# wangtong627/COR

Measured on AMD Instinct MI355X. Metric: query triplets/sec (forward + similarity + top-k), higher is better.
Workload: dtype bf16

## Files before the change

cor_amd/_native.py:

```python
from __future__ import annotations

import ctypes as C
import os

_HERE = os.path.dirname(os.path.abspath(__file__))
LIB_PATH = os.environ.get("COR_AMD_LIB") or os.path.join(_HERE, "csrc", "libcor_amd.so")

F32, BF16, F16, BF16X3 = 0, 1, 2, 3
I8 = 4
ACT_NONE, ACT_GELU_ERF, ACT_RELU, ACT_SIGMOID, ACT_GELU_TANH = 0, 1, 2, 3, 4
EINVAL, ENOSUPPORT = -1, -2
TOPK_FORCE_LISTS, TOPK_NO_FALLBACK, TOPK_FORCE_GLOBAL_THRESHOLD, TOPK_WAVE_FINAL = 1, 2, 8, 16
TOPK_KMAX = 256
FILTER_EQ, FILTER_NE = 0, 1
MERGE_NMAX = 4096
EXPAND_SEGMAX = 16
RERANK_SEGMAX = 16
DIVERSIFY_SEGMAX = 16
DIFFUSE_NMAX, DIFFUSE_KDMAX, DIFFUSE_SEGMAX = 256, 32, 16
CLUSTER_SEGMAX, KMEANS_KMAX = 16, 16384
IVF_NPROBE_MAX = 256
FUSE_PMAX = 16
FUSE_RRF, FUSE_SUM, FUSE_MAX = 0, 1, 2
FUSE_NORM_NONE, FUSE_NORM_MINMAX = 0, 1
FUSE_MISSING_ZERO, FUSE_MISSING_FLOOR = 0, 1
ORDER_REVERSE = 1 << 30
GEMM_KERNEL_SCALAR, GEMM_KERNEL_MASK, GEMM_EPILOGUE_VEC = 32, 0xff, 1 << 8
KERNEL_ROWLANE, KERNEL_FEWQ, KERNEL_FLASH_MFMA, KERNEL_FLASH_PIPELINED, KERNEL_WINDOW_BLOCK = 1, 2, 3, 4, 5
import numpy as _np
Q_PRESCALE_HD64 = float(_np.float32(0.125) * _np.float32(1.4426950408889634))

_p, _i, _l, _f, _ll = C.c_void_p, C.c_int, C.c_long, C.c_float, C.c_longlong

SIGNATURES = {
    "cor_version": [],
    "cor_gemm": [_p, _l, _p, _l, _i, _p, _l, _i, _i, _i, _i, _p, _i, _p, _p, _l, _i, _i, _p],
    "cor_gemm_kernel_id": [_p, _l, _p, _l, _i, _p, _l, _i, _i, _i, _i, _p, _i, _p, _p, _l, _i, _i],
    "cor_layernorm": [_p, _i, _p, _i, _p, _p, _i, _i, _f, _i, _p],
    "cor_attention": [_p, _l, _l, _p, _l, _l, _p, _l, _l, _i, _p, _l, _l, _i, _i, _i, _i, _i, _i, _f, _p],
    "cor_attention_f32": [_p, _l, _l, _p, _l, _l, _p, _l, _l, _p, _l, _l, _i, _i, _i, _i, _i, _i, _f, _p],
    "cor_attention_kernel_id": [_i, _i, _i, _i, _i, _i],
    "cor_sam_attention": [_p, _i, _p, _i, _p, _p, _p, _i, _i, _i, _i, _i, _f, _i, _p],
    "cor_patchify": [_p, _p, _i, _i, _i, _i, _i, _i, _i, _p],
    "cor_im2col3x3": [_p, _i, _p, _i, _i, _i, _i, _p],
    "cor_add": [_p, _i, _p, _i, _p, _i, _l, _l, _p],
    "cor_copy_rows": [_p, _l, _i, _p, _l, _i, _i, _i, _p],
    "cor_split_x3": [_p, _l, _p, _l, _l, _i, _i, _p],
    "cor_tokens_to_nchw": [_p, _i, _p, _i, _i, _i, _p],
    "cor_nchw_to_tokens": [_p, _p, _i, _i, _i, _i, _p],
    "cor_l2norm_rows": [_p, _i, _p, _i, _i, _i, _f, _p],
    "cor_embed_tokens": [_p, _p, _p, _p, _i, _i, _i, _i, _p],
    "cor_bilinear": [_p, _p, _i, _i, _i, _i, _i, _i, _p],
    "cor_conv3x3s2_small": [_p, _i, _p, _p, _p, _i, _i, _i, _i, _i, _p],
    "cor_dwconv7x7": [_p, _p, _p, _p, _i, _i, _i, _i, _i, _p],
    "cor_adapter_pool": [_p, _p, _p, _i, _i, _i, _i, _p],
    "cor_masked_pool": [_p, _i, _p, _p, _i, _i, _i, _i, _i, _p],
    "cor_region_pool": [_p, _p, _p, _p, _i, _i, _i, _i, _i, _i, _i, _p],
    "cor_fuse_gate": [_p, _p, _p, _p, _p, _i, _i, _p],
    "cor_fuse_mix": [_p, _p, _p, _i, _i, _p],
    "cor_dense_pe": [_p, _p, _i, _i, _p],
# ... 100 lines not shown
```

cor_amd/csrc/common.h:

```cpp
#pragma once
#include <hip/hip_runtime.h>
#include <atomic>
#include <stdint.h>

#include "../../include/cor_amd.h"

typedef uint16_t bf16_t;

typedef float f32x4 __attribute__((ext_vector_type(4)));
typedef unsigned int u32x4 __attribute__((ext_vector_type(4)));
typedef float f32x16 __attribute__((ext_vector_type(16)));
typedef __bf16 bf16x8 __attribute__((ext_vector_type(8)));

#define COR_CHECK_LAUNCH()                                  \
  do {                                                      \
    hipError_t e__ = hipGetLastError();                     \
    if (e__ != hipSuccess) return (int)e__;                 \
  } while (0)

__device__ __forceinline__ float bf2f(bf16_t v) { return __uint_as_float(((uint32_t)v) << 16); }
__device__ __forceinline__ bf16_t f2bf(float f) {
  __bf16 b = (__bf16)f;
  return __builtin_bit_cast(uint16_t, b);
}
// ... 80 lines not shown
__device__ __forceinline__ float sigmoid_f(float x) { return 1.0f / (1.0f + __expf(-x)); }

__device__ __forceinline__ float apply_act(float v, int act) {
  switch (act) {
    case COR_ACT_GELU_ERF: return gelu_erf_f(v);
    case COR_ACT_RELU: return fmaxf(v, 0.0f);
    case COR_ACT_SIGMOID: return 1.0f / (1.0f + expf(-v));
    case COR_ACT_GELU_TANH: return gelu_tanh_f(v);
    default: return v;
  }
}

__device__ __forceinline__ float wave_sum(float v) {
#pragma unroll
  for (int o = 32; o > 0; o >>= 1) v += __shfl_xor(v, o, 64);
  return v;
}
__device__ __forceinline__ float wave_max(float v) {
#pragma unroll
  for (int o = 32; o > 0; o >>= 1) v = fmaxf(v, __shfl_xor(v, o, 64));
  return v;
}

__device__ __forceinline__ int xcd_remap(int bid, int nwg) {
  const int xcd = bid & 7, q = nwg >> 3, r = nwg & 7;
  return (xcd < r ? xcd * (q + 1) : r * (q + 1) + (xcd - r) * q) + (bid >> 3);
}

__device__ __forceinline__ void glds16(const void* gsrc, unsigned lds_dst) {
  unsigned keep;
  asm volatile("s_mov_b32 %0, m0\n\ts_mov_b32 m0, %2\n\ts_nop 0\n\tglobal_load_lds_dwordx4 %1, off\n\ts_mov_b32 m0, %0"
               : "=&s"(keep) : "v"(gsrc), "s"(lds_dst) : "memory");
}

__device__ __forceinline__ void glds16_so(const void* sbase, unsigned voff, unsigned lds_dst) {
  unsigned keep;
  asm volatile("s_mov_b32 %0, m0\n\ts_mov_b32 m0, %3\n\ts_nop 0\n\tglobal_load_lds_dwordx4 %1, %2\n\ts_mov_b32 m0, %0"
               : "=&s"(keep) : "v"(voff), "s"(sbase), "s"(lds_dst) : "memory");
}

__device__ __forceinline__ void glds16_so_pair4k(const void* sbase, unsigned voff0_plus2k, unsigned voff1_minus2k, unsigned lds_dst_plus2k) {
  unsigned keep;
  asm volatile("s_mov_b32 %0, m0\n\ts_mov_b32 m0, %4\n\ts_nop 0\n\t"
               "global_load_lds_dwordx4 %1, %3 offset:-2048\n\tglobal_load_lds_dwordx4 %2, %3 offset:2048\n\ts_mov_b32 m0, %0"
               : "=&s"(keep) : "v"(voff0_plus2k), "v"(voff1_minus2k), "s"(sbase), "s"(lds_dst_plus2k) : "memory");
}
// ... 35 lines not shown
```

cor_amd/csrc/gemm.hip:

```cpp
#include "common.h"

#ifdef COR_PROBES
#define COR_DBG(g_, bit_) ((g_).dbg & (bit_))
#else
#define COR_DBG(g_, bit_) 0
#endif
#ifndef COR_GEMM_DEFAULT_BIG
#define COR_GEMM_DEFAULT_BIG 2
#endif

namespace {

struct GemmArgs {
  const char* A; const char* W; char* C;
  long lda_b, ldw_b;
  long ldc;
  int M, N, Kb;
  int tm, tn;
  const float* bias; const float* col_scale; const float* residual;
  long ldr; int res_row_mod; int act;
  int group_m;
  unsigned long long* stamps;
  int dbg;
  int vec_epi;
  int rev;
  int nt_c;
  int order;
};

template <typename TA> struct Mfma;
template <> struct Mfma<float> {
  static __device__ __forceinline__ void run(const uint4& a, const uint4& b, f32x16& acc) {
    acc = __builtin_amdgcn_mfma_f32_32x32x2f32(__uint_as_float(a.x), __uint_as_float(b.x), acc, 0, 0, 0);
    acc = __builtin_amdgcn_mfma_f32_32x32x2f32(__uint_as_float(a.y), __uint_as_float(b.y), acc, 0, 0, 0);
    acc = __builtin_amdgcn_mfma_f32_32x32x2f32(__uint_as_float(a.z), __uint_as_float(b.z), acc, 0, 0, 0);
    acc = __builtin_amdgcn_mfma_f32_32x32x2f32(__uint_as_float(a.w), __uint_as_float(b.w), acc, 0, 0, 0);
  }
};
template <> struct Mfma<bf16_t> {
  static __device__ __forceinline__ void run(const uint4& a, const uint4& b, f32x16& acc) {
    acc = __builtin_amdgcn_mfma_f32_32x32x16_bf16(__builtin_bit_cast(bf16x8, a), __builtin_bit_cast(bf16x8, b), acc, 0, 0, 0);
  }
};

__device__ __forceinline__ void mfma16_bf16(const uint4& a, const uint4& b, f32x4& acc) {
  acc = __builtin_amdgcn_mfma_f32_16x16x32_bf16(__builtin_bit_cast(bf16x8, a), __builtin_bit_cast(bf16x8, b), acc, 0, 0, 0);
}

constexpr int ROWB = 128;

template <int ACT, typename TO = float> __device__ __forceinline__ float act_ct(float v) {
// ... 639 lines not shown
#pragma unroll
        for (int i = 0; i < 8; ++i)
#pragma unroll
          for (int j = 0; j < 4; ++j) t += acc16[i][j][0] + acc16[i][j][3];
      } else {
#pragma unroll
        for (int i = 0; i < MI; ++i)
#pragma unroll
          for (int j = 0; j < NJ; ++j) t += acc[i][j][0] + acc[i][j][15];
      }
      if (t == 1.2345f) ((float*)g.C)[tid] = t;
    } else
    switch (g.act) {
      case COR_ACT_GELU_ERF: COR_EPI(COR_ACT_GELU_ERF) break;
      case COR_ACT_RELU: COR_EPI(COR_ACT_RELU) break;
      case COR_ACT_SIGMOID: COR_EPI(COR_ACT_SIGMOID) break;
      case COR_ACT_GELU_TANH: COR_EPI(COR_ACT_GELU_TANH) break;
      default: COR_EPI(COR_ACT_NONE) break;
    }
#undef COR_EPI
#ifdef COR_PROBES
    if (g.stamps && blockIdx.x == 0 && tid == 0) { g.stamps[(qi - 1) * 16 + 15] = __builtin_readcyclecounter(); g.stamps[(qi - 1) * 16 + 14] = __builtin_amdgcn_s_memrealtime(); }
#endif
    if (Ln < 0) break;
    L = Ln;
    stores_pending = !COR_DBG(g, 2);
  }
}

template <typename TA, typename TO>
__global__ void __launch_bounds__(256) gemm_nt_small(const TA* A, long lda, const TA* W, long ldw, TO* C, long ldc,
                                                     int M, int N, int K, const float* bias, int act,
                                                     const float* col_scale, const float* residual, long ldr,
                                                     int res_row_mod) {
  __shared__ float As[32][33], Ws[32][33];
  const int tx = threadIdx.x & 31, ty = threadIdx.x >> 5;
  const int m0 = blockIdx.y * 32, n0 = blockIdx.x * 32;
  float acc[4] = {0, 0, 0, 0};
  for (int k0 = 0; k0 < K; k0 += 32) {
#pragma unroll
    for (int i = 0; i < 4; ++i) {
      const int rrow = ty + 8 * i, k = k0 + tx;
      As[rrow][tx] = (m0 + rrow < M && k < K) ? ld<TA>(A + (long)(m0 + rrow) * lda + k) : 0.0f;
      Ws[rrow][tx] = (n0 + rrow < N && k < K) ? ld<TA>(W + (long)(n0 + rrow) * ldw + k) : 0.0f;
    }
    __syncthreads();
#pragma unroll 8
    for (int kk = 0; kk < 32; ++kk) {
      const float w = Ws[tx][kk];
// ... 49 lines not shown
  if (cfg == 0) {
    cfg = (k128 && M >= 512 && N >= 64) ? ((N <= 256 && K >= 2048 && M >= 65536) ? 9 : COR_GEMM_DEFAULT_BIG) : 1;
    if (k128 && M < 512 && N >= 64) cfg = 4;
    if (cfg == 2 && (long)cdiv(M, 128) * cdiv(N, 128) < 256) cfg = 4;
    else if (cfg == 2 && (long)cdiv(M, 128) * cdiv(N, 128) < 512) cfg = 3;
    if (sizeof(TA) == 2 && k128 && !col_scale && (long)cdiv(M, 256) * cdiv(N, 256) >= 140 && 4L * N >= 3L * 256 * cdiv(N, 256) && K >= 256) cfg = 13;
  }
  if (!k128 && (cfg == 2 || cfg == 3 || cfg == 4)) cfg = 1;
  if (cfg == 13 || cfg == 14) {
    const long c_bytes = (((long)M - 1) * ldc + N) * (long)sizeof(TO);
    const bool ok = sizeof(TA) == 2 && k128 && vec_epi && !col_scale && N % 8 == 0 && c_bytes < (1L << 32) - 64 && !(sizeof(TO) == 2 && residual) &&
                    (long)M * lda_b < (1L << 32) && (long)N * ldw_b < (1L << 32);
    if (!ok) cfg = k128 ? 2 : 1;
    else return {cfg, vec_epi};
  }
  if (!k128 && cfg >= 9) cfg = 1;
  if (!(cfg == 9 || cfg == 2 || cfg == 3 || cfg == 4)) cfg = 1;
  return {cfg, vec_epi};
}

template <typename TA, typename TO>
int launch_gemm(const void* A, long lda, const void* W, long ldw, void* C, long ldc, int M, int N, int K,
                const float* bias, int act, const float* col_scale, const float* residual, long ldr, int res_row_mod,
                int cfg_arg, hipStream_t s) {
  const int g_gemm_dbg = (cfg_arg & ~COR_ORDER_REVERSE) >> 8;
  const long esz = sizeof(TA);
  const GemmRoute route = gemm_route<TA, TO>(A, lda, W, ldw, C, ldc, M, N, K, bias, col_scale, residual, ldr, cfg_arg);
  if (route.kernel == COR_GEMM_KERNEL_SCALAR) {
    hipLaunchKernelGGL((gemm_nt_small<TA, TO>), dim3(cdiv(N, 32), cdiv(M, 32)), dim3(256), 0, s, (const TA*)A, lda,
                       (const TA*)W, ldw, (TO*)C, ldc, M, N, K, bias, act, col_scale, residual, ldr, res_row_mod);
    COR_CHECK_LAUNCH();
    return 0;
  }
  GemmArgs g;
  g.A = (const char*)A; g.W = (const char*)W; g.C = (char*)C;
  g.lda_b = lda * esz; g.ldw_b = ldw * esz; g.ldc = ldc;
  g.M = M; g.N = N; g.Kb = (int)(K * esz);
  g.stamps = nullptr;
#ifdef COR_PROBES
  if (g_gemm_dbg & 0x100000) { g.stamps = (unsigned long long*)col_scale; col_scale = nullptr; }
#endif
  g.bias = bias; g.col_scale = col_scale; g.residual = residual; g.ldr = ldr; g.res_row_mod = res_row_mod; g.act = act;
  g.dbg = g_gemm_dbg & 0x3fefff; g.rev = (cfg_arg & COR_ORDER_REVERSE) ? 1 : 0;
  g.order = 1;
  g.nt_c = (sizeof(TO) == 2 && !residual) ? 1 : 0;
  g.group_m = ((g_gemm_dbg >> 4) & 0xff) ? ((g_gemm_dbg >> 4) & 0xff) : 8;
  g.vec_epi = route.vec_epi;
  const int cfg = route.kernel;
  if (cfg == 13 || cfg == 14) {
    if constexpr (sizeof(TA) == 2) {
      g.tm = cdiv(g.M, 256); g.tn = cdiv(g.N, 256);
      g.order = g.tn <= 4 ? 1 : 0;
      if (g_gemm_dbg & 0x1000) g.order ^= 1;
      static DevOnce once_a;
      const int n_cu = cor_device_cus();
      cor_max_dyn_lds((const void*)gemm_pp<TO, false>, 163840, once_a);
#ifdef COR_PROBES
      static DevOnce once_b;
      cor_max_dyn_lds((const void*)gemm_pp<TO, true>, 163840, once_b);
#endif
      const int total = g.tm * g.tn;
      int blocks = n_cu - (n_cu & 7);
      if (total < blocks) blocks = ((total + 7) / 8) * 8;
#ifdef COR_PROBES
      if (cfg == 14) hipLaunchKernelGGL((gemm_pp<TO, true>), dim3(blocks), dim3(512), 163840, s, g);
      else
#endif
      hipLaunchKernelGGL((gemm_pp<TO, false>), dim3(blocks), dim3(512), 163840, s, g);
      COR_CHECK_LAUNCH();
      return 0;
    }
  }
  switch (cfg) {
    case 9: return launch_tile<TA, TO, 256, 128, 4, 2, true, 3>(g, s);
    case 2: return launch_tile<TA, TO, 128, 128, 2, 2, true>(g, s);
    case 3: return launch_tile<TA, TO, 128, 64, 2, 2, true>(g, s);
    case 4: return launch_tile<TA, TO, 64, 64, 2, 2, true>(g, s);
    default: return launch_tile<TA, TO, 128, 128, 2, 2, false>(g, s);
  }
}

int gemm_check_args(const void* A, long lda, const void* W, long ldw, int& ab_dtype, const void* C, long ldc, int c_dtype, int M, int N, int& K,
                    const float* residual, long ldr, int cfg) {
  if (!A || !W || !C || M <= 0 || N <= 0 || K <= 0 || lda < K || ldw < K || ldc < N) return COR_EINVAL;
  {
    const int sel = cfg & 0xff;
// ... 23 lines not shown
  hipStream_t s = (hipStream_t)stream;
  if (ab_dtype == COR_F32 && c_dtype == COR_F32)
    return launch_gemm<float, float>(A, lda, W, ldw, C, ldc, M, N, K, bias, act, col_scale, residual, ldr, res_row_mod, cfg, s);
  if (ab_dtype == COR_BF16 && c_dtype == COR_BF16)
    return launch_gemm<bf16_t, bf16_t>(A, lda, W, ldw, C, ldc, M, N, K, bias, act, col_scale, residual, ldr, res_row_mod, cfg, s);
  if (ab_dtype == COR_BF16 && c_dtype == COR_F32)
    return launch_gemm<bf16_t, float>(A, lda, W, ldw, C, ldc, M, N, K, bias, act, col_scale, residual, ldr, res_row_mod, cfg, s);
  return launch_gemm<float, bf16_t>(A, lda, W, ldw, C, ldc, M, N, K, bias, act, col_scale, residual, ldr, res_row_mod, cfg, s);
}

extern "C" int cor_gemm_kernel_id(const void* A, long lda, const void* W, long ldw, int ab_dtype, const void* C, long ldc, int c_dtype,
                                  int M, int N, int K, const float* bias, int act, const float* col_scale,
                                  const float* residual, long ldr, int res_row_mod, int cfg) {
  (void)act; (void)res_row_mod;
  const int rc = gemm_check_args(A, lda, W, ldw, ab_dtype, C, ldc, c_dtype, M, N, K, residual, ldr, cfg);
  if (rc) return rc;
  GemmRoute r;
  if (ab_dtype == COR_F32 && c_dtype == COR_F32) r = gemm_route<float, float>(A, lda, W, ldw, C, ldc, M, N, K, bias, col_scale, residual, ldr, cfg);
  else if (ab_dtype == COR_BF16 && c_dtype == COR_BF16) r = gemm_route<bf16_t, bf16_t>(A, lda, W, ldw, C, ldc, M, N, K, bias, col_scale, residual, ldr, cfg);
  else if (ab_dtype == COR_BF16 && c_dtype == COR_F32) r = gemm_route<bf16_t, float>(A, lda, W, ldw, C, ldc, M, N, K, bias, col_scale, residual, ldr, cfg);
  else r = gemm_route<float, bf16_t>(A, lda, W, ldw, C, ldc, M, N, K, bias, col_scale, residual, ldr, cfg);
  return r.kernel | (r.vec_epi ? COR_GEMM_EPILOGUE_VEC : 0);
}
```

cor_amd/csrc/rows.hip:

```cpp
#include "common.h"

namespace {

template <typename TI, typename TO, int MAXV>
__global__ void __launch_bounds__(256) layernorm_kernel(const TI* x, TO* y, const float* w, const float* b, int rows, int C,
                                                        float eps, int act, int rev) {
  const int lane = threadIdx.x & 63;
  const int row = (rev ? (int)gridDim.x - 1 - (int)blockIdx.x : (int)blockIdx.x) * 4 + (threadIdx.x >> 6);
  if (row >= rows) return;
  const TI* xr = x + (long)row * C;
  const int nv = C >> 2;
  f32x4 v[MAXV];
  float s = 0.f;
#pragma unroll
  for (int i = 0; i < MAXV; ++i) {
    const int j = lane + 64 * i;
    if (j < nv) { v[i] = ld4<TI>(xr + 4 * j); s += v[i][0] + v[i][1] + v[i][2] + v[i][3]; }
  }
  const float mean = wave_sum(s) / C;
  float q = 0.f;
#pragma unroll
  for (int i = 0; i < MAXV; ++i) {
    const int j = lane + 64 * i;
    if (j < nv) {
// ... 1 lines not shown
      for (int e = 0; e < 4; ++e) { const float d = v[i][e] - mean; q += d * d; }
    }
  }
  const float rstd = 1.0f / sqrtf(wave_sum(q) / C + eps);
#pragma unroll
  for (int i = 0; i < MAXV; ++i) {
    const int j = lane + 64 * i;
    if (j < nv) {
      const f32x4 wv = *(const f32x4*)(w + 4 * j), bv = *(const f32x4*)(b + 4 * j);
      f32x4 o;
#pragma unroll
      for (int e = 0; e < 4; ++e) o[e] = apply_act((v[i][e] - mean) * rstd * wv[e] + bv[e], act);
      st4_row<TO>(y, row, C, 4 * j, o);
    }
  }
}

template <typename TI, typename TO, int NV, bool NT>
__global__ void __launch_bounds__(256) layernorm_half_kernel(const TI* x, TO* y, const float* w, const float* b, int rows, int C,
                                                             float eps, int act, int rev) {
  const int lane = threadIdx.x & 31;
  const int row = (rev ? (int)gridDim.x - 1 - (int)blockIdx.x : (int)blockIdx.x) * 8 + (threadIdx.x >> 5);
  if (row >= rows) return;
  const TI* xr = x + (long)row * C;
  f32x4 v[NV];
  float s = 0.f;
#pragma unroll
  for (int i = 0; i < NV; ++i) {
    if constexpr (NT && sizeof(TI) == 4) v[i] = __builtin_nontemporal_load((const f32x4*)(xr + 4 * (lane + 32 * i)));
    else v[i] = ld4<TI>(xr + 4 * (lane + 32 * i));
    s += (v[i][0] + v[i][1]) + (v[i][2] + v[i][3]);
  }
  auto hsum = [](float t) {
#pragma unroll
    for (int o = 16; o > 0; o >>= 1) t += __shfl_xor(t, o, 64);
    return t;
  };
  const float mean = hsum(s) / C;
  float q = 0.f;
#pragma unroll
  for (int i = 0; i < NV; ++i)
#pragma unroll
    for (int e = 0; e < 4; ++e) { const float d = v[i][e] - mean; q += d * d; }
  const float rstd = 1.0f / sqrtf(hsum(q) / C + eps);
#pragma unroll
  for (int i = 0; i < NV; ++i) {
    const int j = lane + 32 * i;
    const f32x4 wv = *(const f32x4*)(w + 4 * j), bv = *(const f32x4*)(b + 4 * j);
    f32x4 o;
#pragma unroll
    for (int e = 0; e < 4; ++e) o[e] = apply_act((v[i][e] - mean) * rstd * wv[e] + bv[e], act);
    st4_row<TO>(y, row, C, 4 * j, o);
  }
}

#ifdef COR_PROBES
template <int NV, bool WRITE_X>
__global__ void __launch_bounds__(256) layernorm_delta_probe(float* x, const bf16_t* dl, bf16_t* y, const float* w, const float* b, int rows, int C, float eps) {
  const int lane = threadIdx.x & 31;
  const int row = ((int)gridDim.x - 1 - (int)blockIdx.x) * 8 + (threadIdx.x >> 5);
  if (row >= rows) return;
  float* xr = x + (long)row * C;
  const bf16_t* dr = dl + (long)row * C;
  f32x4 v[NV];
  float s = 0.f;
#pragma unroll
  for (int i = 0; i < NV; ++i) {
    v[i] = __builtin_nontemporal_load((const f32x4*)(xr + 4 * (lane + 32 * i)));
    const f32x4 d = ld4<bf16_t>(dr + 4 * (lane + 32 * i));
    v[i] += d;
    if (WRITE_X) *(f32x4*)(xr + 4 * (lane + 32 * i)) = v[i];
    s += (v[i][0] + v[i][1]) + (v[i][2] + v[i][3]);
  }
  auto hsum = [](float t) {
#pragma unroll
    for (int o = 16; o > 0; o >>= 1) t += __shfl_xor(t, o, 64);
// ... 375 lines not shown
```

cor_amd/engine.py:

```python
from __future__ import annotations

import math

import torch

from . import _native as nat
from . import ops
from .ops import ACT_NONE, ACT_GELU_ERF, ACT_RELU, ACT_SIGMOID, ACT_GELU_TANH, X3

F32 = torch.float32


def _round_up(x, m):
    return (x + m - 1) // m * m


class _Packer:

    def __init__(self, sd: dict, T: torch.dtype):
        dev = next(iter(sd.values())).device
        if dev.type != "cuda":
            raise RuntimeError("cor_amd: the model must live on a GPU (model.to('cuda')); there is no CPU path")
        self.sd, self.T, self.W = sd, T, {}

# ... 137 lines not shown

def pack(sd: dict, scfg: dict, gcfg: dict, mask_pooling: str, T: torch.dtype, Q=None) -> dict:
    pk = _Packer(sd, T)
    pkq = pk if Q is None or Q == T else _Packer(sd, Q)
    pack_sam_encoder(pk, scfg)
    pack_prompt_encoder(pk)
    pack_siglip(pkq, gcfg)
    pack_support_head(pkq, mask_pooling)
    pack_mask_decoder(pk)
    if pkq is not pk:
        pk.W.update(pkq.W)
    return pk.W


def _lin(W, p, a, out_dtype, act=ACT_NONE, residual=None, col_scale=None, out=None, reverse=False, x3=False):
    return ops.gemm(a, W[p + "weight"], out_dtype=out_dtype, bias=W[p + "bias"], act=act, residual=residual,
                    col_scale=col_scale, out=out, reverse=reverse, x3=x3)


def _ln(W, p, x, eps, out_dtype, act=ACT_NONE, reverse=False):
    return ops.layernorm(x, W[p + "weight"], W[p + "bias"], eps, out_dtype=out_dtype, act=act, reverse=reverse)


def _gelu(kind):
    return ACT_GELU_ERF if kind == "erf" else ACT_GELU_TANH


def sam_encoder(W, img, cfg, T, p="image_encoder."):
    B = img.shape[0]
    g, d, H = cfg["img"] // cfg["patch"], cfg["dim"], cfg["heads"]
    assert img.shape[1:] == (3, cfg["img"], cfg["img"]), f"SAM input must be [B,3,{cfg['img']},{cfg['img']}], got {tuple(img.shape)}"
    cols = ops.patchify(img, cfg["patch"], W[p + "patch.K"], T)
    x = ops.gemm(cols, W[p + "patch_embed.proj.weight"], out_dtype=F32, bias=W[p + "patch_embed.proj.bias"],
                 residual=W[p + "pos_embed"], res_row_mod=g * g)
    del cols
    for i in range(cfg["depth"]):
        b = f"{p}blocks.{i}."
        win = 0 if i in cfg["global_idx"] else cfg["window"]
        h = _ln(W, b + "norm1.", x, 1e-6, T, reverse=True)
        qkv = _lin(W, b + "attn.qkv.", h, T)
        a = ops.sam_attention(qkv, W[b + "attn.pad_row"], W[b + "attn.rel_pos_h"], W[b + "attn.rel_pos_w"], B, H, g, win,
                              q_prescale=W[b + "attn.q_prescale"], reverse=True)
        del qkv
        _lin(W, b + "attn.proj.", a, F32, residual=x, out=x)
        h = _ln(W, b + "norm2.", x, 1e-6, T, reverse=True)
        m = _lin(W, b + "mlp.lin1.", h, T, act=ACT_GELU_ERF)
        _lin(W, b + "mlp.lin2.", m, F32, residual=x, out=x)
        del h, a, m
    y = ops.gemm(ops.cast(x, T), W[p + "neck.0.weight"], out_dtype=F32)
    y = _ln(W, p + "neck.1.", y, 1e-6, T)
    y = ops.gemm(ops.im2col3x3(y, B, g, g), W[p + "neck.2.weight"], out_dtype=F32)
    return _ln(W, p + "neck.3.", y, 1e-6, F32)


def _vit_mha(qkv, N, Tn, heads, D, T):
    hd = D // heads
    if T == X3:
        return ops.attention_f32(qkv[:, 0:D], qkv[:, D:2 * D], qkv[:, 2 * D:3 * D], N, heads, Tn, Tn, hd, hd ** -0.5, out_dtype=X3)
    return ops.attention(qkv[:, 0:D], qkv[:, D:2 * D], qkv[:, 2 * D:3 * D], N, heads, Tn, Tn, hd, hd ** -0.5, out_dtype=T)


def _qkv_dtype(T):
    return F32 if T == X3 else T


def siglip_vision(W, img, g, T, p="support_branch.siglip.model.visual.trunk."):
    N = img.shape[0]
    D, P = g["dim"], (g["image"] // g["patch"]) ** 2
    x3 = T == X3
    assert img.shape[1:] == (3, g["image"], g["image"]), f"SigLIP input must be [N,3,{g['image']},{g['image']}], got {tuple(img.shape)}"
    cols = ops.patchify(img, g["patch"], W[p + "patch.K"], T)
    x = ops.gemm(cols, W[p + "patch_embed.proj.weight"], out_dtype=F32, bias=W[p + "patch_embed.proj.bias"],
                 residual=W[p + "pos_embed"], res_row_mod=P, x3=x3)
    act = _gelu(g.get("v_gelu", g.get("gelu", "erf")))
    for i in range(g["depth"]):
        b = f"{p}blocks.{i}."
        h = _ln(W, b + "norm1.", x, 1e-6, T)
        qkv = _lin(W, b + "attn.qkv.", h, _qkv_dtype(T), x3=x3)
        a = _vit_mha(qkv, N, P, g["heads"], D, T)
        _lin(W, b + "attn.proj.", a, F32, residual=x, out=x, x3=x3)
        h = _ln(W, b + "norm2.", x, 1e-6, T)
        m = _lin(W, b + "mlp.fc1.", h, T, act=act, x3=x3)
        _lin(W, b + "mlp.fc2.", m, F32, residual=x, out=x, x3=x3)
    return _ln(W, p + "norm.", x, 1e-6, F32)


def siglip_text(W, tokens, g, T, p="support_branch.siglip.model.text."):
    N, ctx = tokens.shape
    D = g["dim"]
    x3 = T == X3
    x = ops.embed_tokens(tokens.contiguous(), W[p + "token_embedding.weight"], W[p + "positional_embedding"])
    act = _gelu(g.get("t_gelu", g.get("gelu", "erf")))
    for i in range(g["t_depth"]):
        b = f"{p}transformer.resblocks.{i}."
        h = _ln(W, b + "ln_1.", x, 1e-6, T)
        qkv = ops.gemm(h, W[b + "attn.in_proj_weight"], out_dtype=_qkv_dtype(T), bias=W[b + "attn.in_proj_bias"], x3=x3)
        a = _vit_mha(qkv, N, ctx, g["t_heads"], D, T)
        _lin(W, b + "attn.out_proj.", a, F32, residual=x, out=x, x3=x3)
        h = _ln(W, b + "ln_2.", x, 1e-6, T)
        m = _lin(W, b + "mlp.c_fc.", h, T, act=act, x3=x3)
        _lin(W, b + "mlp.c_proj.", m, F32, residual=x, out=x, x3=x3)
    last = torch.empty((N, D), dtype=F32, device=x.device)
    ops.copy_rows(x, ctx * D, N, D, last, src_offset=(ctx - 1) * D)
    last = _ln(W, p + "ln_final.", last, 1e-6, T)
    feat = _lin(W, p + "text_projection.", last, F32, x3=x3)
    return ops.l2norm_rows(feat)
# ... 217 lines not shown
```

cor_amd/ops.py:

```python
from __future__ import annotations

import math

import torch

from . import _native as nat
from ._native import ACT_NONE, ACT_GELU_ERF, ACT_RELU, ACT_SIGMOID, ACT_GELU_TANH, F32, BF16, F16

_DT = {torch.float32: F32, torch.bfloat16: BF16, torch.float16: F16}

X3 = "bf16x3"

GEMM_PROFILE = None


def _lib():
    return nat.load()


def _dt(t: torch.Tensor) -> int:
    return _DT[t.dtype]


def _s():
    return torch.cuda.current_stream().cuda_stream


def _p(t):
    return 0 if t is None else t.data_ptr()


def _dev(*ts):
    dev = None
    for t in ts:
        if t is None:
            continue
# ... 7 lines not shown
        raise RuntimeError(f"cor_amd ops: operands live on {dev} but the current device is cuda:{torch.cuda.current_device()}; "
                           f"wrap the call in `with torch.cuda.device({dev.index})`")
    return dev


def _rows(t: torch.Tensor):
    assert t.dim() == 2 and t.stride(1) == 1, f"expected 2-D row-major view, got {tuple(t.shape)} / {t.stride()}"
    return t.shape[0], t.shape[1], t.stride(0) if t.shape[0] > 1 else max(t.stride(0), t.shape[1])


def _f32vec(t, n, name):
    if t is None:
        return
    assert t.dtype == torch.float32 and t.is_contiguous() and t.numel() == n, f"{name}: need contiguous fp32[{n}]"


def split_weight_x3(w):
    w = w.detach().to(torch.float32)
    hi = w.to(torch.bfloat16)
    lo = (w - hi.to(torch.float32)).to(torch.bfloat16)
    return torch.cat([hi, lo, hi], dim=1).contiguous()


def gemm(a, w, out_dtype=None, bias=None, act=ACT_NONE, col_scale=None, residual=None, res_row_mod=0, out=None, cfg=0, reverse=False,
         x3=False):
    if out_dtype == X3:
        assert out is None and x3
        y = gemm(a, w, torch.float32, bias, act, col_scale, residual, res_row_mod, None, cfg, reverse, x3)
        return split_x3(y)
    _dev(a, w, bias, col_scale, residual, out)
    M, K, lda = _rows(a)
    N, K2, ldw = _rows(w)
    assert K == K2 and a.dtype == w.dtype, (a.shape, w.shape, a.dtype, w.dtype)
    if x3:
        assert a.dtype == torch.bfloat16 and K % 3 == 0, (a.shape, a.dtype)
        K //= 3
    if out is None:
        out = torch.empty((M, N), dtype=out_dtype or a.dtype, device=a.device)
    Mo, No, ldc = _rows(out)
    assert (Mo, No) == (M, N)
    _f32vec(bias, N, "bias")
    _f32vec(col_scale, N, "col_scale")
    ldr = 0
    if residual is not None:
        Mr, Nr, ldr = _rows(residual)
        assert residual.dtype == torch.float32 and Nr == N and Mr == (res_row_mod if res_row_mod > 0 else M)
    prof = GEMM_PROFILE
    if prof is not None:
        e0, e1 = torch.cuda.Event(enable_timing=True), torch.cuda.Event(enable_timing=True)
        e0.record()
    nat.check(_lib().cor_gemm(a.data_ptr(), lda, w.data_ptr(), ldw, nat.BF16X3 if x3 else _dt(a), out.data_ptr(), ldc, _dt(out), M, N, K,
                              _p(bias), act, _p(col_scale), _p(residual), ldr, res_row_mod, int(cfg) | (nat.ORDER_REVERSE if reverse else 0), _s()), "cor_gemm")
    if prof is not None:
        e1.record()
        k_run = 3 * K if x3 else K
        nbytes = (M * k_run + N * k_run) * a.element_size() + M * N * out.element_size() + (M * N * 4 if residual is not None else 0)
        prof.append((e0, e1, 2.0 * M * N * k_run, a.dtype, float(nbytes)))
    return out


def layernorm(x, w, b, eps, out_dtype=None, act=ACT_NONE, out=None, reverse=False):
    _dev(x, w, b, out)
    assert x.is_contiguous() and x.dim() == 2
    rows, C = x.shape
    _f32vec(w, C, "ln.weight")
    _f32vec(b, C, "ln.bias")
    if out_dtype == X3:
        assert out is None and x.dtype == torch.float32
        out = torch.empty((rows, 3 * C), dtype=torch.bfloat16, device=x.device)
        y_dt = nat.BF16X3
    else:
        if out is None:
            out = torch.empty((rows, C), dtype=out_dtype or x.dtype, device=x.device)
        assert out.is_contiguous() and out.shape == x.shape
        y_dt = _dt(out)
    nat.check(_lib().cor_layernorm(x.data_ptr(), _dt(x), out.data_ptr(), y_dt, w.data_ptr(), b.data_ptr(), rows, C,
                                   float(eps), act | (nat.ORDER_REVERSE if reverse else 0), _s()), "cor_layernorm")
    return out


def _attn_out(out, rows, cols, dtype, device, strided):
# ... 1102 lines not shown
```

include/cor_amd.h:

```cpp
#ifndef COR_AMD_H
#define COR_AMD_H

#ifdef __cplusplus
extern "C" {
#endif

#define COR_EINVAL (-1)
#define COR_ENOSUPPORT (-2)
#define COR_ORDER_REVERSE (1 << 30)
#define COR_TOPK_FORCE_LISTS 1
#define COR_TOPK_NO_FALLBACK 2
#define COR_TOPK_FORCE_GLOBAL_THRESHOLD 8
#define COR_TOPK_WAVE_FINAL 16
#define COR_TOPK_KMAX 256
#define COR_MERGE_NMAX 4096
#define COR_FILTER_EQ 0
#define COR_FILTER_NE 1

enum { COR_F32 = 0, COR_BF16 = 1, COR_F16 = 2 , COR_BF16X3 = 3 ,
       COR_I8 = 4  };
enum { COR_ACT_NONE = 0, COR_ACT_GELU_ERF = 1, COR_ACT_RELU = 2, COR_ACT_SIGMOID = 3, COR_ACT_GELU_TANH = 4 };

int cor_version(void);


int cor_gemm(const void* A, long lda, const void* W, long ldw, int ab_dtype,
             void* C, long ldc, int c_dtype, int M, int N, int K,
             const float* bias, int act, const float* col_scale,
             const float* residual, long ldr, int res_row_mod, int cfg, void* stream);

#define COR_GEMM_KERNEL_SCALAR 32
#define COR_GEMM_KERNEL_MASK 0xff
#define COR_GEMM_EPILOGUE_VEC (1 << 8)
int cor_gemm_kernel_id(const void* A, long lda, const void* W, long ldw, int ab_dtype,
                       const void* C, long ldc, int c_dtype, int M, int N, int K,
                       const float* bias, int act, const float* col_scale,
                       const float* residual, long ldr, int res_row_mod, int cfg);

int cor_layernorm(const void* x, int x_dtype, void* y, int y_dtype, const float* w, const float* b,
                  int rows, int C, float eps, int act, void* stream);


int cor_attention(const void* q, long q_sb, long q_st, const void* k, long k_sb, long k_st,
                  const void* v, long v_sb, long v_st, int dtype,
                  void* out, long o_sb, long o_st, int out_dtype,
                  int B, int H, int Tq, int Tk, int hd, float scale, void* stream);

int cor_attention_f32(const float* q, long q_sb, long q_st, const float* k, long k_sb, long k_st,
                      const float* v, long v_sb, long v_st, void* out, long o_sb, long o_st, int out_dtype,
                      int B, int H, int Tq, int Tk, int hd, float scale, void* stream);

int cor_sam_attention(const void* qkv, int dtype, void* out, int out_dtype, const void* pad_row,
                      const float* rel_h, const float* rel_w, int B, int H, int hd, int grid, int window, float q_prescale, int variant,
                      void* stream);

enum { COR_KERNEL_ROWLANE = 1, COR_KERNEL_FEWQ = 2, COR_KERNEL_FLASH_MFMA = 3, COR_KERNEL_FLASH_PIPELINED = 4, COR_KERNEL_WINDOW_BLOCK = 5 };
int cor_attention_kernel_id(int dtype, int hd, int Tq, int Tk, int sam_window, int grid);


int cor_patchify(const float* img, void* out, int out_dtype, int B, int C, int H, int W, int p, int Kpad, void* stream);

// ... 186 lines not shown
```

Baseline: 776.4.

## Fuse residual-GEMM with following LayerNorm via per-row-block arrival counters

Adds a fused GEMM+LayerNorm path. The last workgroup to finish a BM-row block, detected through an atomic counter, computes LayerNorm (or a plain cast) on the fp32 residual stream and writes bf16 output. The ViT and SAM encoder loops now use it for proj and MLP-out GEMMs, removing separate layernorm launches and one re-read of the residual. It only applies to the persistent kernel route with N=768, and it adds an atomic/fence step plus serial tail work inside the GEMM.

```diff
diff --git a/cor_amd/_native.py b/cor_amd/_native.py
--- a/cor_amd/_native.py
+++ b/cor_amd/_native.py
@@ -36,6 +36,7 @@
     "cor_version": [],
     "cor_gemm": [_p, _l, _p, _l, _i, _p, _l, _i, _i, _i, _i, _p, _i, _p, _p, _l, _i, _i, _p],
     "cor_gemm_kernel_id": [_p, _l, _p, _l, _i, _p, _l, _i, _i, _i, _i, _p, _i, _p, _p, _l, _i, _i],
+    "cor_gemm_ln": [_p, _l, _p, _l, _p, _l, _i, _i, _i, _p, _i, _p, _l, _i, _i, _p, _p, _f, _p, _p, _i, _p],
     "cor_layernorm": [_p, _i, _p, _i, _p, _p, _i, _i, _f, _i, _p],
     "cor_attention": [_p, _l, _l, _p, _l, _l, _p, _l, _l, _i, _p, _l, _l, _i, _i, _i, _i, _i, _i, _f, _p],
     "cor_attention_f32": [_p, _l, _l, _p, _l, _l, _p, _l, _l, _p, _l, _l, _i, _i, _i, _i, _i, _i, _f, _p],
diff --git a/cor_amd/csrc/common.h b/cor_amd/csrc/common.h
--- a/cor_amd/csrc/common.h
+++ b/cor_amd/csrc/common.h
@@ -126,6 +126,45 @@
   return v;
 }
 
+template <typename TI, typename TO, int NV, bool NT, bool CAST = false>
+__device__ __forceinline__ void ln_half_row(const TI* xr, TO* y, long row, const float* w, const float* b, int C, float eps, int act, int lane) {
+#pragma clang fp contract(off)
+  f32x4 v[NV];
+  float s = 0.f;
+#pragma unroll
+  for (int i = 0; i < NV; ++i) {
+    if constexpr (NT && sizeof(TI) == 4) v[i] = __builtin_nontemporal_load((const f32x4*)(xr + 4 * (lane + 32 * i)));
+    else v[i] = ld4<TI>(xr + 4 * (lane + 32 * i));
+    s += (v[i][0] + v[i][1]) + (v[i][2] + v[i][3]);
+  }
+  if constexpr (CAST) {
+#pragma unroll
+    for (int i = 0; i < NV; ++i) st4_row<TO>(y, row, C, 4 * (lane + 32 * i), v[i]);
+    return;
+  }
+  auto hsum = [](float t) {
+#pragma unroll
+    for (int o = 16; o > 0; o >>= 1) t += __shfl_xor(t, o, 64);
+    return t;
+  };
+  const float mean = hsum(s) / C;
+  float q = 0.f;
+#pragma unroll
+  for (int i = 0; i < NV; ++i)
+#pragma unroll
+    for (int e = 0; e < 4; ++e) { const float d = v[i][e] - mean; q = fmaf(d, d, q); }
+  const float rstd = 1.0f / sqrtf(hsum(q) / C + eps);
+#pragma unroll
+  for (int i = 0; i < NV; ++i) {
+    const int j = lane + 32 * i;
+    const f32x4 wv = *(const f32x4*)(w + 4 * j), bv = *(const f32x4*)(b + 4 * j);
+    f32x4 o;
+#pragma unroll
+    for (int e = 0; e < 4; ++e) o[e] = apply_act(fmaf((v[i][e] - mean) * rstd, wv[e], bv[e]), act);
+    st4_row<TO>(y, row, C, 4 * j, o);
+  }
+}
+
 __device__ __forceinline__ int xcd_remap(int bid, int nwg) {
   const int xcd = bid & 7, q = nwg >> 3, r = nwg & 7;
   return (xcd < r ? xcd * (q + 1) : r * (q + 1) + (xcd - r) * q) + (bid >> 3);
diff --git a/cor_amd/csrc/gemm.hip b/cor_amd/csrc/gemm.hip
--- a/cor_amd/csrc/gemm.hip
+++ b/cor_amd/csrc/gemm.hip
@@ -26,7 +26,10 @@
   int rev;
   int nt_c;
   int order;
+  const float* ln_w; const float* ln_b; float ln_eps; bf16_t* ln_out; int* ln_cnt;
 };
+
+struct LnTail { const float* w; const float* b; float eps; void* out; int* cnt; int test_grid; };
 
 template <typename TA> struct Mfma;
 template <> struct Mfma<float> {
@@ -712,9 +715,37 @@
 #ifdef COR_PROBES
     if (g.stamps && blockIdx.x == 0 && tid == 0) { g.stamps[(qi - 1) * 16 + 15] = __builtin_readcyclecounter(); g.stamps[(qi - 1) * 16 + 14] = __builtin_amdgcn_s_memrealtime(); }
 #endif
+    bool published = false;
+    if constexpr (sizeof(TO) == 4 && !M16) {
+      if (g.ln_out) {
+        COR_VMCNT(0);
+        __syncthreads();
+        int* flag = (int*)(smem + 4 * HT);
+        int* cnt = g.ln_cnt + cm0 / BM;
+        const int wv = (int)(wslot >> 10);
+        const int ln64 = (int)__builtin_amdgcn_mbcnt_hi(~0u, __builtin_amdgcn_mbcnt_lo(~0u, 0u));
+        const bool first = wv == 0 && ln64 == 0;
+        if (first) *flag = __hip_atomic_fetch_add(cnt, 1, __ATOMIC_ACQ_REL, __HIP_MEMORY_SCOPE_AGENT);
+        __syncthreads();
+        const bool owner = *flag == g.tn - 1;
+        if (owner) {
+          if (first) __hip_atomic_store(cnt, 0, __ATOMIC_RELAXED, __HIP_MEMORY_SCOPE_AGENT);
+          __builtin_amdgcn_fence(__ATOMIC_ACQUIRE, "agent");
+          const int hw = 2 * wv + (ln64 >> 5), l32 = ln64 & 31;
+          const float* xc = (const float*)g.C;
+          const int rend = min(BM, g.M - cm0);
+          for (int rr = hw; rr < rend; rr += 16) {
+            const long row = cm0 + rr;
+            if (g.ln_w) ln_half_row<float, bf16_t, 6, false, false>(xc + row * g.ldc, g.ln_out, row, g.ln_w, g.ln_b, g.N, g.ln_eps, COR_ACT_NONE, l32);
+            else ln_half_row<float, bf16_t, 6, false, true>(xc + row * g.ldc, g.ln_out, row, nullptr, nullptr, g.N, 0.f, COR_ACT_NONE, l32);
+          }
+        }
+        published = true;
+      }
+    }
     if (Ln < 0) break;
     L = Ln;
-    stores_pending = !COR_DBG(g, 2);
+    stores_pending = !COR_DBG(g, 2) && !published;
   }
 }
 
@@ -810,10 +841,11 @@
 template <typename TA, typename TO>
 int launch_gemm(const void* A, long lda, const void* W, long ldw, void* C, long ldc, int M, int N, int K,
                 const float* bias, int act, const float* col_scale, const float* residual, long ldr, int res_row_mod,
-                int cfg_arg, hipStream_t s) {
+                int cfg_arg, hipStream_t s, const LnTail* ln = nullptr) {
   const int g_gemm_dbg = (cfg_arg & ~COR_ORDER_REVERSE) >> 8;
   const long esz = sizeof(TA);
   const GemmRoute route = gemm_route<TA, TO>(A, lda, W, ldw, C, ldc, M, N, K, bias, col_scale, residual, ldr, cfg_arg);
+  if (ln && !(route.kernel == 13 && sizeof(TA) == 2 && sizeof(TO) == 4)) return COR_EINVAL;
   if (route.kernel == COR_GEMM_KERNEL_SCALAR) {
     hipLaunchKernelGGL((gemm_nt_small<TA, TO>), dim3(cdiv(N, 32), cdiv(M, 32)), dim3(256), 0, s, (const TA*)A, lda,
                        (const TA*)W, ldw, (TO*)C, ldc, M, N, K, bias, act, col_scale, residual, ldr, res_row_mod);
@@ -834,6 +866,7 @@
   g.nt_c = (sizeof(TO) == 2 && !residual) ? 1 : 0;
   g.group_m = ((g_gemm_dbg >> 4) & 0xff) ? ((g_gemm_dbg >> 4) & 0xff) : 8;
   g.vec_epi = route.vec_epi;
+  g.ln_w = nullptr; g.ln_b = nullptr; g.ln_eps = 0.f; g.ln_out = nullptr; g.ln_cnt = nullptr;
   const int cfg = route.kernel;
   if (cfg == 13 || cfg == 14) {
     if constexpr (sizeof(TA) == 2) {
@@ -850,6 +883,14 @@
       const int total = g.tm * g.tn;
       int blocks = n_cu - (n_cu & 7);
       if (total < blocks) blocks = ((total + 7) / 8) * 8;
+      if (ln) {
+        if (g.order != 1 || g.N != 768 || !residual) return COR_EINVAL;
+        if (ln->test_grid > 0) {
+          if ((ln->test_grid & 7) || ln->test_grid > n_cu - (n_cu & 7)) return COR_EINVAL;
+          blocks = ln->test_grid;
+        }
+        g.ln_w = ln->w; g.ln_b = ln->b; g.ln_eps = ln->eps; g.ln_out = (bf16_t*)ln->out; g.ln_cnt = ln->cnt;
+      }
 #ifdef COR_PROBES
       if (cfg == 14) hipLaunchKernelGGL((gemm_pp<TO, true>), dim3(blocks), dim3(512), 163840, s, g);
       else
@@ -919,3 +960,19 @@
   else r = gemm_route<float, bf16_t>(A, lda, W, ldw, C, ldc, M, N, K, bias, col_scale, residual, ldr, cfg);
   return r.kernel | (r.vec_epi ? COR_GEMM_EPILOGUE_VEC : 0);
 }
+
+extern "C" int cor_gemm_ln(const void* A, long lda, const void* W, long ldw, void* C, long ldc, int M, int N, int K, const float* bias, int act,
+                           const float* residual, long ldr, int res_row_mod, int cfg, const float* ln_w, const float* ln_b, float ln_eps,
+                           void* ln_out, int* ln_cnt, int test_grid, void* stream) {
+  int ab = COR_BF16;
+  const int rc = gemm_check_args(A, lda, W, ldw, ab, C, ldc, COR_F32, M, N, K, residual, ldr, cfg);
+  if (rc) return rc;
+  if (!ln_out || !ln_cnt || !residual || N != 768 || (ln_w == nullptr) != (ln_b == nullptr) || test_grid < 0) return COR_EINVAL;
+  if (((uintptr_t)ln_out & 7) || (ln_w && (((uintptr_t)ln_w | (uintptr_t)ln_b) & 15)) || ldc % 4 != 0 || ((uintptr_t)C & 15)) return COR_EINVAL;
+  if (ln_out == C || ln_out == (const void*)residual) return COR_EINVAL;
+  const int sel = cfg & 0xff;
+  if (!(sel == 0 || sel == 13)) return COR_EINVAL;
+  if (test_grid > 0) cfg = (cfg & ~0xff) | 13;
+  const LnTail ln{ln_w, ln_b, ln_eps, ln_out, ln_cnt, test_grid};
+  return launch_gemm<bf16_t, float>(A, lda, W, ldw, C, ldc, M, N, K, bias, act, nullptr, residual, ldr, res_row_mod, cfg, (hipStream_t)stream, &ln);
+}
diff --git a/cor_amd/csrc/rows.hip b/cor_amd/csrc/rows.hip
--- a/cor_amd/csrc/rows.hip
+++ b/cor_amd/csrc/rows.hip
@@ -47,36 +47,7 @@
   const int lane = threadIdx.x & 31;
   const int row = (rev ? (int)gridDim.x - 1 - (int)blockIdx.x : (int)blockIdx.x) * 8 + (threadIdx.x >> 5);
   if (row >= rows) return;
-  const TI* xr = x + (long)row * C;
-  f32x4 v[NV];
-  float s = 0.f;
-#pragma unroll
-  for (int i = 0; i < NV; ++i) {
-    if constexpr (NT && sizeof(TI) == 4) v[i] = __builtin_nontemporal_load((const f32x4*)(xr + 4 * (lane + 32 * i)));
-    else v[i] = ld4<TI>(xr + 4 * (lane + 32 * i));
-    s += (v[i][0] + v[i][1]) + (v[i][2] + v[i][3]);
-  }
-  auto hsum = [](float t) {
-#pragma unroll
-    for (int o = 16; o > 0; o >>= 1) t += __shfl_xor(t, o, 64);
-    return t;
-  };
-  const float mean = hsum(s) / C;
-  float q = 0.f;
-#pragma unroll
-  for (int i = 0; i < NV; ++i)
-#pragma unroll
-    for (int e = 0; e < 4; ++e) { const float d = v[i][e] - mean; q += d * d; }
-  const float rstd = 1.0f / sqrtf(hsum(q) / C + eps);
-#pragma unroll
-  for (int i = 0; i < NV; ++i) {
-    const int j = lane + 32 * i;
-    const f32x4 wv = *(const f32x4*)(w + 4 * j), bv = *(const f32x4*)(b + 4 * j);
-    f32x4 o;
-#pragma unroll
-    for (int e = 0; e < 4; ++e) o[e] = apply_act((v[i][e] - mean) * rstd * wv[e] + bv[e], act);
-    st4_row<TO>(y, row, C, 4 * j, o);
-  }
+  ln_half_row<TI, TO, NV, NT>(x + (long)row * C, y, row, w, b, C, eps, act, lane);
 }
 
 #ifdef COR_PROBES
diff --git a/cor_amd/engine.py b/cor_amd/engine.py
--- a/cor_amd/engine.py
+++ b/cor_amd/engine.py
@@ -183,6 +183,15 @@
     return ops.layernorm(x, W[p + "weight"], W[p + "bias"], eps, out_dtype=out_dtype, act=act, reverse=reverse)
 
 
+FUSE_LN_TAIL = True
+
+
+def _lin_ln(W, p, a, x, norm, eps, T, cnt, reverse=False, x3=False):
+    ln = (None, None, 0.0) if norm is None else (W[norm + "weight"], W[norm + "bias"], eps)
+    return ops.gemm(a, W[p + "weight"], out_dtype=F32, bias=W[p + "bias"], residual=x, out=x, x3=x3, ln=ln, ln_dtype=T, ln_cnt=cnt,
+                    ln_reverse=reverse, ln_fuse=FUSE_LN_TAIL)
+
+
 def _gelu(kind):
     return ACT_GELU_ERF if kind == "erf" else ACT_GELU_TANH
 
@@ -195,20 +204,21 @@
     x = ops.gemm(cols, W[p + "patch_embed.proj.weight"], out_dtype=F32, bias=W[p + "patch_embed.proj.bias"],
                  residual=W[p + "pos_embed"], res_row_mod=g * g)
     del cols
+    cnt = ops.ln_counters(x.shape[0], x.device)
+    h = _ln(W, f"{p}blocks.0.norm1.", x, 1e-6, T, reverse=True)
     for i in range(cfg["depth"]):
         b = f"{p}blocks.{i}."
         win = 0 if i in cfg["global_idx"] else cfg["window"]
-        h = _ln(W, b + "norm1.", x, 1e-6, T, reverse=True)
         qkv = _lin(W, b + "attn.qkv.", h, T)
         a = ops.sam_attention(qkv, W[b + "attn.pad_row"], W[b + "attn.rel_pos_h"], W[b + "attn.rel_pos_w"], B, H, g, win,
                               q_prescale=W[b + "attn.q_prescale"], reverse=True)
         del qkv
-        _lin(W, b + "attn.proj.", a, F32, residual=x, out=x)
-        h = _ln(W, b + "norm2.", x, 1e-6, T, reverse=True)
+        h = _lin_ln(W, b + "attn.proj.", a, x, b + "norm2.", 1e-6, T, cnt, reverse=True)
         m = _lin(W, b + "mlp.lin1.", h, T, act=ACT_GELU_ERF)
-        _lin(W, b + "mlp.lin2.", m, F32, residual=x, out=x)
-        del h, a, m
-    y = ops.gemm(ops.cast(x, T), W[p + "neck.0.weight"], out_dtype=F32)
+        nxt = f"{p}blocks.{i + 1}.norm1." if i + 1 < cfg["depth"] else None
+        h = _lin_ln(W, b + "mlp.lin2.", m, x, nxt, 1e-6, T, cnt, reverse=True)
+        del a, m
+    y = ops.gemm(h, W[p + "neck.0.weight"], out_dtype=F32)
     y = _ln(W, p + "neck.1.", y, 1e-6, T)
     y = ops.gemm(ops.im2col3x3(y, B, g, g), W[p + "neck.2.weight"], out_dtype=F32)
     return _ln(W, p + "neck.3.", y, 1e-6, F32)
@@ -234,15 +244,18 @@
     x = ops.gemm(cols, W[p + "patch_embed.proj.weight"], out_dtype=F32, bias=W[p + "patch_embed.proj.bias"],
                  residual=W[p + "pos_embed"], res_row_mod=P, x3=x3)
     act = _gelu(g.get("v_gelu", g.get("gelu", "erf")))
+    cnt = ops.ln_counters(x.shape[0], x.device)
+    h = _ln(W, f"{p}blocks.0.norm1.", x, 1e-6, T)
     for i in range(g["depth"]):
         b = f"{p}blocks.{i}."
-        h = _ln(W, b + "norm1.", x, 1e-6, T)
         qkv = _lin(W, b + "attn.qkv.", h, _qkv_dtype(T), x3=x3)
         a = _vit_mha(qkv, N, P, g["heads"], D, T)
-        _lin(W, b + "attn.proj.", a, F32, residual=x, out=x, x3=x3)
-        h = _ln(W, b + "norm2.", x, 1e-6, T)
+        h = _lin_ln(W, b + "attn.proj.", a, x, b + "norm2.", 1e-6, T, cnt, x3=x3)
         m = _lin(W, b + "mlp.fc1.", h, T, act=act, x3=x3)
-        _lin(W, b + "mlp.fc2.", m, F32, residual=x, out=x, x3=x3)
+        if i + 1 < g["depth"]:
+            h = _lin_ln(W, b + "mlp.fc2.", m, x, f"{p}blocks.{i + 1}.norm1.", 1e-6, T, cnt, x3=x3)
+        else:
+            _lin(W, b + "mlp.fc2.", m, F32, residual=x, out=x, x3=x3)
     return _ln(W, p + "norm.", x, 1e-6, F32)
 
 
diff --git a/cor_amd/ops.py b/cor_amd/ops.py
--- a/cor_amd/ops.py
+++ b/cor_amd/ops.py
@@ -12,6 +12,7 @@
 X3 = "bf16x3"
 
 GEMM_PROFILE = None
+FUSED_LN_LAUNCHES = 0
 
 
 def _lib():
@@ -65,8 +66,16 @@
     return torch.cat([hi, lo, hi], dim=1).contiguous()
 
 
+def ln_counters(rows, device):
+    return torch.zeros((max(1, (int(rows) + 255) // 256),), dtype=torch.int32, device=device)
+
+
 def gemm(a, w, out_dtype=None, bias=None, act=ACT_NONE, col_scale=None, residual=None, res_row_mod=0, out=None, cfg=0, reverse=False,
-         x3=False):
+         x3=False, ln=None, ln_out=None, ln_dtype=None, ln_cnt=None, ln_reverse=False, ln_fuse=True, _test_grid=0):
+    if ln is not None:
+        return _gemm_ln(a, w, out_dtype, bias, act, col_scale, residual, res_row_mod, out, cfg, reverse, x3, ln, ln_out, ln_dtype, ln_cnt,
+                        ln_reverse, ln_fuse, _test_grid)
+    assert ln_out is None and _test_grid == 0
     if out_dtype == X3:
         assert out is None and x3
         y = gemm(a, w, torch.float32, bias, act, col_scale, residual, res_row_mod, None, cfg, reverse, x3)
@@ -100,6 +109,56 @@
         nbytes = (M * k_run + N * k_run) * a.element_size() + M * N * out.element_size() + (M * N * 4 if residual is not None else 0)
         prof.append((e0, e1, 2.0 * M * N * k_run, a.dtype, float(nbytes)))
     return out
+
+
+def _gemm_ln(a, w, out_dtype, bias, act, col_scale, residual, res_row_mod, out, cfg, reverse, x3, ln, ln_out, ln_dtype, ln_cnt, ln_reverse,
+             ln_fuse, test_grid):
+    lw, lb, eps = ln
+    assert out is not None and (lw is None) == (lb is None)
+    ln_dtype = ln_dtype or a.dtype
+    _dev(a, w, bias, col_scale, residual, out, lw, lb, ln_out, ln_cnt)
+    M, K, lda = _rows(a)
+    N, K2, ldw = _rows(w)
+    fused = (ln_fuse and not x3 and a.dtype == torch.bfloat16 and w.dtype == torch.bfloat16 and out.dtype == torch.float32 and
+             ln_dtype == torch.bfloat16 and residual is not None and col_scale is None and N == 768 and K == K2 and int(cfg) in (0, 13))
+    if fused:
+        Mo, No, ldc = _rows(out)
+        Mr, Nr, ldr = _rows(residual)
+        assert (Mo, No) == (M, N) and residual.dtype == torch.float32 and Nr == N and Mr == (res_row_mod if res_row_mod > 0 else M)
+        if test_grid == 0:
+            kid = _lib().cor_gemm_kernel_id(a.data_ptr(), lda, w.data_ptr(), ldw, BF16, out.data_ptr(), ldc, F32, M, N, K, _p(bias), act, 0,
+                                            residual.data_ptr(), ldr, res_row_mod, int(cfg))
+            fused = kid >= 0 and (kid & nat.GEMM_KERNEL_MASK) == 13
+    if not fused:
+        assert test_grid == 0, "gemm(ln=..., _test_grid): these operands do not take the fused route"
+        gemm(a, w, out_dtype, bias, act, col_scale, residual, res_row_mod, out, cfg, reverse, x3)
+        if lw is None:
+            assert ln_out is None
+            return cast(out, ln_dtype)
+        return layernorm(out, lw, lb, eps, out_dtype=ln_dtype, out=ln_out, reverse=ln_reverse)
+    _f32vec(bias, N, "bias")
+    _f32vec(lw, N, "ln.weight")
+    _f32vec(lb, N, "ln.bias")
+    if ln_out is None:
+        ln_out = torch.empty((M, N), dtype=torch.bfloat16, device=a.device)
+    assert ln_out.dtype == torch.bfloat16 and ln_out.is_contiguous() and tuple(ln_out.shape) == (M, N)
+    if ln_cnt is None:
+        ln_cnt = ln_counters(M, a.device)
+    assert ln_cnt.dtype == torch.int32 and ln_cnt.is_contiguous() and ln_cnt.numel() >= (M + 255) // 256
+    global FUSED_LN_LAUNCHES
+    FUSED_LN_LAUNCHES += 1
+    prof = GEMM_PROFILE
+    if prof is not None:
+        e0, e1 = torch.cuda.Event(enable_timing=True), torch.cuda.Event(enable_timing=True)
+        e0.record()
+    nat.check(_lib().cor_gemm_ln(a.data_ptr(), lda, w.data_ptr(), ldw, out.data_ptr(), ldc, M, N, K, _p(bias), act, residual.data_ptr(), ldr,
+                                 res_row_mod, int(cfg) | (nat.ORDER_REVERSE if reverse else 0), _p(lw), _p(lb), float(eps), ln_out.data_ptr(),
+                                 ln_cnt.data_ptr(), int(test_grid), _s()), "cor_gemm_ln")
+    if prof is not None:
+        e1.record()
+        nbytes = (M * K + N * K) * a.element_size() + M * N * 4 + M * N * 4 + M * N * 2
+        prof.append((e0, e1, 2.0 * M * N * K, a.dtype, float(nbytes)))
+    return ln_out
 
 
 def layernorm(x, w, b, eps, out_dtype=None, act=ACT_NONE, out=None, reverse=False):
diff --git a/include/cor_amd.h b/include/cor_amd.h
--- a/include/cor_amd.h
+++ b/include/cor_amd.h
@@ -37,6 +37,10 @@
                        const float* bias, int act, const float* col_scale,
                        const float* residual, long ldr, int res_row_mod, int cfg);
 
+int cor_gemm_ln(const void* A, long lda, const void* W, long ldw, void* C, long ldc, int M, int N, int K,
+                const float* bias, int act, const float* residual, long ldr, int res_row_mod, int cfg,
+                const float* ln_w, const float* ln_b, float ln_eps, void* ln_out, int* ln_cnt, int test_grid, void* stream);
+
 int cor_layernorm(const void* x, int x_dtype, void* y, int y_dtype, const float* w, const float* b,
                   int rows, int C, float eps, int act, void* stream);
 
```

New measurement: 674.7. -13.1%, worse.
